# xxcclong/Distributed-CUDA-BFS

Measured on AMD Instinct MI355X. Metric: GTEPS (traversed edges/sec) on RMAT-26 + soc-LiveJournal1 at 1/2/4/8 MI355X, higher is better.
Workload: dtype uint8 levels (int32 on read)

## Files before the change

csrc/backend/cpu_backend.cpp:

```cpp
#include <algorithm>
#include <chrono>
#include <cstdlib>
#include <cstring>
#include <utility>
#include <vector>

#include "dbfs/backend.hpp"

namespace dbfs {
namespace {

inline void put_level(lvl_t* wide, uint8_t* narrow, int64_t i, lvl_t level, uint8_t base) {
  if (narrow) narrow[i] = static_cast<uint8_t>(base + (level <= kNarrowMaxLevel ? level : kNarrowMaxLevel + 1));
  else wide[i] = level;
}

inline bool test_bit(const word_t* bm, uint64_t v) { return (bm[v >> 6] >> (v & 63)) & 1ull; }
inline word_t gather_bytes(uint8_t* p) {
  word_t bits = 0;
  for (int b = 0; b < 64; ++b)
    if (p[b]) bits |= 1ull << b;
  if (bits) std::memset(p, 0, 64);
  return bits;
}
// ... 618 lines not shown
  void encode_hub_cols(const vid_t* col, int64_t nnz, const uint32_t* hub_idx, vid_t* out) override {
    for (int64_t e = 0; e < nnz; ++e) out[e] = hub_idx[col[e]] != 0xFFFFFFFFu ? (kHubFlag | hub_idx[col[e]]) : col[e];
  }
  void nz_word_counts(const eid_t* ro, int64_t rows, int64_t words, eid_t* counts) override {
    for (int64_t w = 0; w < words; ++w) {
      eid_t c = 0;
      for (int64_t v = w * 64; v < std::min<int64_t>(rows, (w + 1) * 64); ++v) c += ro[v + 1] > ro[v] ? 1 : 0;
      counts[w] = c;
    }
  }
  void nz_fill(const eid_t* ro, const vid_t* head, int64_t rows, const eid_t* pref, eid_t* nz_ro,
               vid_t* nz_head) override {
    int64_t k = 0;
    for (int64_t v = 0; v < rows; ++v) {
      if (ro[v + 1] > ro[v]) {
        nz_ro[k] = ro[v];
        nz_head[k] = head[v];
        ++k;
      }
    }
    nz_ro[k] = rows > 0 ? ro[rows] : 0;
    (void)pref;
  }
  void nz_records(const eid_t* ro, const vid_t* head, int64_t rows, const eid_t* pref, NzRec* rec,
                  eid_t* unit_base) override {
    const int64_t nunits = div_up(std::max<int64_t>(rows, 1), kUnitVertices);
    for (int64_t u = 0; u <= nunits; ++u) unit_base[u] = ro[std::min<int64_t>(u * kUnitVertices, rows)];
    int64_t k = 0;
    for (int64_t v = 0; v < rows; ++v) {
      if (ro[v + 1] > ro[v]) {
        rec[k].off = static_cast<uint32_t>(ro[v] - unit_base[v / kUnitVertices]);
        rec[k].head = head[v];
        ++k;
      }
    }
    (void)pref;
  }
  int64_t select_hubs(const uint32_t* deg, int64_t n, uint32_t min_deg, vid_t* hub_vertex,
                      uint32_t* hub_idx) override {
    int64_t k = 0;
    for (int64_t v = 0; v < n; ++v) {
      if (deg[v] >= min_deg) {
        hub_vertex[k] = static_cast<vid_t>(v);
        hub_idx[v] = static_cast<uint32_t>(k++);
      } else {
        hub_idx[v] = 0xFFFFFFFFu;
      }
    }
    return k;
  }
  void hub_gather(const HubGatherArgs& a) override {
    if (a.ctrl && (a.ctrl->done || a.ctrl->dir != 'B')) return;
    for (int64_t w = 0; w < div_up(a.g.nhubs, 64); ++w) {
      word_t m = 0;
      int64_t d = 0;
// ... 193 lines not shown
```

csrc/backend/hip_backend.cpp:

```cpp
#include <hip/hip_runtime.h>

#include <chrono>
#include <cstdlib>
#include <cstring>
#include <string>
#include <vector>

#include "dbfs/backend.hpp"
#include "../kernels/launch.hpp"

namespace dbfs {

#define HIP_CHECK(expr)                                                                              \
  do {                                                                                               \
    hipError_t e_ = (expr);                                                                          \
    if (e_ != hipSuccess)                                                                            \
      ::dbfs::raise_error(__FILE__, __LINE__, std::string("HIP error ") + hipGetErrorString(e_) +    \
                                                  " in " #expr);                                     \
  } while (0)

namespace {

class HipBackend final : public Backend {
 public:
// ... 241 lines not shown
  void validate_levels(const ValidateArgs& a) override { on(); kern::validate_levels(a, st_); chk(); }
  void compute_parents(const ParentArgs& a) override { on(); kern::compute_parents(a, st_); chk(); }
  void degrees_u32(const eid_t* ro, int64_t rows, uint32_t* out) override {
    on();
    kern::degrees_u32(ro, rows, out, st_);
    chk();
  }
  void row_heads(const eid_t* ro, const vid_t* col, int64_t rows, vid_t* head, const uint32_t* hub_idx) override {
    on();
    kern::row_heads(ro, col, rows, head, hub_idx, st_);
    chk();
  }

  void encode_hub_cols(const vid_t* col, int64_t nnz, const uint32_t* hub_idx, vid_t* out) override {
    on();
    kern::encode_hub_cols(col, nnz, hub_idx, out, st_);
    chk();
  }
  void nz_word_counts(const eid_t* ro, int64_t rows, int64_t words, eid_t* counts) override {
    on();
    kern::nz_word_counts(ro, rows, words, counts, st_);
    chk();
  }
  void nz_records(const eid_t* ro, const vid_t* head, int64_t rows, const eid_t* pref, NzRec* rec,
                  eid_t* unit_base) override {
    on();
    kern::nz_records(ro, head, rows, div_up(rows, kWordBits), pref, rec, unit_base, st_);
    chk();
  }
  void nz_fill(const eid_t* ro, const vid_t* head, int64_t rows, const eid_t* pref, eid_t* nz_ro,
               vid_t* nz_head) override {
    on();
    kern::nz_fill(ro, head, rows, div_up(rows, kWordBits), pref, nz_ro, nz_head, st_);
    chk();
  }
  int64_t select_hubs(const uint32_t* deg, int64_t n, uint32_t min_deg, vid_t* hub_vertex,
                      uint32_t* hub_idx) override {
    on();
    const int64_t words = div_up(std::max<int64_t>(n, 1), kWordBits);
    eid_t* cnt = nullptr;
    HIP_CHECK(hipMalloc(&cnt, static_cast<size_t>(words + 1) * sizeof(eid_t)));
    HIP_CHECK(hipMemsetAsync(cnt, 0, static_cast<size_t>(words + 1) * sizeof(eid_t), st_));
    kern::hub_count(deg, n, min_deg, cnt, st_);
    chk();
    exclusive_scan(cnt, words);
    kern::hub_assign(deg, n, min_deg, cnt, hub_vertex, hub_idx, st_);
    chk();
    eid_t h = 0;
    HIP_CHECK(hipMemcpyAsync(&h, cnt + words, sizeof(h), hipMemcpyDeviceToHost, st_));
    HIP_CHECK(hipStreamSynchronize(st_));
// ... 124 lines not shown
```

csrc/engine/engine.cpp:

```cpp
#include <algorithm>
#include <chrono>
#include <cstdio>
#include <cstdlib>
#include <cstring>
#include <thread>
#include <vector>

#include "dbfs/engine.hpp"
#include "dbfs/shard_reader.hpp"
#include "dbfs/trace.hpp"
#include "spin.hpp"

namespace dbfs {

Mode parse_mode(const std::string& s) {
  if (s == "ref" || s == "reference") return Mode::Ref;
  if (s == "td" || s == "topdown" || s == "top-down") return Mode::TopDown;
  if (s == "bu" || s == "bottomup" || s == "bottom-up") return Mode::BottomUp;
  if (s == "do" || s == "diropt" || s == "direction-optimizing" || s == "hybrid") return Mode::DirOpt;
  if (s == "simple" || s == "status") return Mode::Simple;
  if (s == "scan") return Mode::Scan;
  throw Error("unknown mode '" + s + "' (expected ref|td|bu|do|simple|scan)");
}

// ... 237 lines not shown
  auto g = from_edges(be, comm, part, rank, es.m, es.u.data(), es.v.data(), es.local_edges());
  g->ingest_ = {es.byte_begin, es.byte_end, es.local_edges()};
  return g;
}

ShardView DeviceGraph::view() const {
  ShardView v;
  v.row_off = row_off_.data();
  v.col = col_.data();
  v.n = part_.n;
  v.lo = lo_;
  v.rows = rows_;
  v.nnz = nnz_;
  v.head = head_.data();
  v.hub_vertex = hub_vertex_.data();
  v.nhubs = nhubs_;
  v.hub_col = hub_col_.data();
  v.hub_bits = hub_bits_.data();
  v.hub_deg = hub_deg_.data();
  v.nz_pref = nz_pref_.data();
  v.nz_row_off = nz_row_off_.data();
  v.nz_head = nz_head_.data();
  v.nz_rec = nz_rec_.data();
  v.unit_base = unit_base_.data();
  if (td_nhubs_ > 0) {
    v.td_col = td_col_.data();
    v.td_hub_vertex = td_hub_vertex_.data();
    v.td_nhubs = td_nhubs_;
  }
  return v;
}

HostCSR DeviceGraph::to_host() const {
  HostCSR h;
  h.n = part_.n;
  h.row_lo = lo_;
  h.rows = rows_;
  h.input_edges = input_edges_;
  h.row_off.resize(static_cast<size_t>(rows_ + 1));
  h.col.resize(static_cast<size_t>(nnz_));
  be_->to_host(h.row_off.data(), row_off_.data(), h.row_off.size() * sizeof(eid_t));
  if (nnz_) be_->to_host(h.col.data(), col_.data(), h.col.size() * sizeof(vid_t));
  return h;
}

std::vector<eid_t> DeviceGraph::degrees_of(const std::vector<int64_t>& local_rows) const {
  std::vector<eid_t> out;
  out.reserve(local_rows.size());
  for (int64_t r : local_rows) {
    DBFS_CHECK(r >= 0 && r < rows_, "row out of range");
    eid_t a[2];
    be_->to_host(a, row_off_.data() + r, sizeof(a));
    out.push_back(a[1] - a[0]);
  }
  return out;
}

static uint32_t hub_min_degree(const std::vector<uint32_t>& deg, int64_t cap) {
  constexpr uint32_t kCapDeg = 1u << 20;
  std::vector<int64_t> hist(kCapDeg + 1, 0);
  for (uint32_t d : deg) ++hist[std::min(d, kCapDeg)];
  int64_t acc = 0;
  uint32_t best = 0;
  for (uint32_t d = kCapDeg; d >= 1; --d) {
    acc += hist[d];
    if (acc > cap) break;
// ... 91 lines not shown
  hub_sorted_ = true;
}

void DeviceGraph::build_heads(const uint32_t* hub_idx) {
  if (head_.size() < static_cast<size_t>(std::max<int64_t>(rows_, 1)))
    head_ = DBuf<vid_t>(*be_, static_cast<size_t>(std::max<int64_t>(rows_, 1)));
  be_->row_heads(row_off_.data(), col_.data(), rows_, head_.data(), hub_idx);
  build_nz_view();
  be_->synchronize();
}

void DeviceGraph::build_nz_view() {
  const int64_t words = div_up(std::max<int64_t>(rows_, 1), kWordBits);
  nz_pref_ = DBuf<eid_t>(*be_, static_cast<size_t>(words + 1));
  be_->memset_async(nz_pref_.data(), 0, nz_pref_.bytes());
  be_->nz_word_counts(row_off_.data(), rows_, words, nz_pref_.data());
  be_->exclusive_scan(nz_pref_.data(), words);
  eid_t nzrows = 0;
  be_->to_host(&nzrows, nz_pref_.data() + words, sizeof(eid_t));
  nz_row_off_ = DBuf<eid_t>(*be_, static_cast<size_t>(nzrows + 1));
  nz_head_ = DBuf<vid_t>(*be_, static_cast<size_t>(std::max<eid_t>(nzrows, 1)));
  be_->nz_fill(row_off_.data(), head_.data(), rows_, nz_pref_.data(), nz_row_off_.data(), nz_head_.data());
  nz_rec_ = DBuf<NzRec>();
  unit_base_ = DBuf<eid_t>();
  if (rows_ <= 0) return;
  const int64_t nunits = div_up(rows_, kUnitVertices);
  unit_base_ = DBuf<eid_t>(*be_, static_cast<size_t>(nunits + 1));
  nz_rec_ = DBuf<NzRec>(*be_, static_cast<size_t>(std::max<eid_t>(nzrows, 1)));
  be_->nz_records(row_off_.data(), head_.data(), rows_, nz_pref_.data(), nz_rec_.data(), unit_base_.data());
  std::vector<eid_t> ub(static_cast<size_t>(nunits + 1));
  be_->to_host(ub.data(), unit_base_.data(), ub.size() * sizeof(eid_t));
  for (int64_t u = 0; u < nunits; ++u)
    if (ub[static_cast<size_t>(u + 1)] - ub[static_cast<size_t>(u)] >= (eid_t(1) << 32)) {
      nz_rec_ = DBuf<NzRec>();
      unit_base_ = DBuf<eid_t>();
      break;
    }
}


Engine::Engine(DeviceGraph& g, Comm& comm, const EngineOptions& opt)
    : g_(g), comm_(comm), be_(g.backend()), opt_(opt), part_(g.partition()), fault_(FaultSpec::from_env()) {
  DBFS_CHECK(comm.size() == part_.nranks, "communicator size does not match the partition");
  DBFS_CHECK(comm.rank() == g.rank(), "communicator rank does not match the shard");
  comm_.bind_backend(&be_);
  total_directed_ = comm_.sum_host(g.nnz());
  level_ = DBuf<lvl_t>(be_, static_cast<size_t>(std::max<int64_t>(g.rows(), 1)));
  be_.fill_level(level_.data(), g.rows(), kUnreached);
}

Engine::~Engine() {
  if (mailbox_host_) be_.free_mapped(mailbox_host_);
  for (auto& seg : rec_segs_) be_.free_mapped(seg.first);
  if (stats_mb_host_) be_.free_mapped(stats_mb_host_);
}


// ... 724 lines not shown
```

csrc/include/dbfs/backend.hpp:

```cpp
#pragma once

#include <atomic>
#include <cstddef>
#include <functional>
#include <memory>
#include <string>
#include <utility>

#include "dbfs/common.hpp"
#include "dbfs/rmat.hpp"

namespace dbfs {

enum class DeviceKind { CPU, HIP };


struct alignas(8) NzRec {
  uint32_t off;
  vid_t head;
};

struct ShardView {
  const eid_t* row_off = nullptr;
  const vid_t* col = nullptr;
  int64_t n = 0, lo = 0, rows = 0, nnz = 0;
  const vid_t* head = nullptr;
  const vid_t* hub_vertex = nullptr;
  int64_t nhubs = 0;
  const vid_t* hub_col = nullptr;
  const eid_t* nz_pref = nullptr;
  const eid_t* nz_row_off = nullptr;
  const vid_t* nz_head = nullptr;
  const struct NzRec* nz_rec = nullptr;
  const eid_t* unit_base = nullptr;
  const vid_t* td_col = nullptr;
  const vid_t* td_hub_vertex = nullptr;
  int64_t td_nhubs = 0;
  const word_t* hub_bits = nullptr;
  const uint32_t* hub_deg = nullptr;
};

#ifndef DBFS_TD_MAX_HUBS_LOG2
#define DBFS_TD_MAX_HUBS_LOG2 16
#endif
constexpr int64_t kTdMaxHubs = int64_t(1) << DBFS_TD_MAX_HUBS_LOG2;

#ifndef DBFS_MAX_HUBS
#define DBFS_MAX_HUBS ((int64_t(1) << 19) - (int64_t(1) << 12))
#endif
constexpr int64_t kMaxHubs = DBFS_MAX_HUBS;
constexpr vid_t kHubFlag = 0x80000000u;
constexpr int kSortedRowMax = 4096;
constexpr uint8_t kNarrowUnreached = 0xFF;
constexpr int kNarrowMaxLevel = 62;
constexpr int kNarrowEpochs = 4;

// ... 604 lines not shown
  virtual bool device_checks_enabled() const { return false; }
  virtual uint64_t take_device_check() { return 0; }
  virtual void inject_device_check() {}
  virtual void status_expand(const StatusArgs& a) = 0;
  virtual void bitmap_or(word_t* dst, const word_t* src, int64_t words) = 0;
  virtual void ref_expand(const RefExpandArgs& a) = 0;
  virtual void ref_accept(const RefAcceptArgs& a) = 0;
  virtual void scan_relax(const ScanBfsArgs& a) = 0;
  virtual void scan_count(const ScanBfsArgs& a) = 0;
  virtual void scan_bounds(const ScanBfsArgs& a) = 0;
  virtual void scan_assign(const ScanBfsArgs& a) = 0;
  virtual void validate_levels(const ValidateArgs& a) = 0;
  virtual void compute_parents(const ParentArgs& a) = 0;

  virtual void degrees_u32(const eid_t* row_off, int64_t rows, uint32_t* out) = 0;
  virtual void sort_neighbors(const eid_t* row_off, vid_t* col, int64_t rows, const uint32_t* key_deg) = 0;
  virtual void sort_rows_by_id(const eid_t* row_off, vid_t* col, int64_t rows, int64_t n) = 0;
  virtual void row_heads(const eid_t* row_off, const vid_t* col, int64_t rows, vid_t* head,
                         const uint32_t* hub_idx = nullptr) = 0;
  virtual void nz_word_counts(const eid_t* row_off, int64_t rows, int64_t words, eid_t* counts) = 0;
  virtual void nz_fill(const eid_t* row_off, const vid_t* head, int64_t rows, const eid_t* nz_pref, eid_t* nz_row_off,
                       vid_t* nz_head) = 0;
  virtual void nz_records(const eid_t* row_off, const vid_t* head, int64_t rows, const eid_t* nz_pref, NzRec* rec,
                          eid_t* unit_base) = 0;
  virtual void encode_hub_cols(const vid_t* col, int64_t nnz, const uint32_t* hub_idx, vid_t* out) = 0;
  virtual int64_t select_hubs(const uint32_t* deg_all, int64_t n, uint32_t min_deg, vid_t* hub_vertex,
                              uint32_t* hub_idx) = 0;

  virtual void gen_count_degrees(const GenParams& p, int64_t lo, int64_t rows, eid_t* deg) = 0;
  virtual void exclusive_scan(eid_t* data, int64_t n) = 0;
  virtual void gen_fill(const GenParams& p, int64_t lo, int64_t rows, eid_t* cursor, vid_t* col) = 0;
  virtual void route_edges_count(const vid_t* u, const vid_t* v, int64_t m, int64_t part, int nranks,
                                 int64_t* counts) = 0;
  virtual void route_edges_fill(const vid_t* u, const vid_t* v, int64_t m, int64_t part, int nranks,
                                int64_t* cursor, uint64_t* out) = 0;
  virtual void entries_count(const uint64_t* e, int64_t k, int64_t lo, eid_t* deg) = 0;
  virtual void entries_fill(const uint64_t* e, int64_t k, int64_t lo, eid_t* cursor, vid_t* col) = 0;
  virtual void reached_degree_sum(const ShardView& g, const lvl_t* level, int64_t* out2) = 0;
  virtual void degree_moments(const ShardView& g, int64_t* out2) = 0;
  virtual void widen_levels(const uint8_t* in, lvl_t* out, int64_t n, uint8_t base) = 0;

 protected:
  std::function<void(double)> wait_watch_;
  double wait_period_ = 0.05;
  std::atomic<int64_t> live_bytes_{0}, peak_bytes_{0};
};

// ... 45 lines not shown
```

csrc/include/dbfs/engine.hpp:

```cpp
#pragma once

#include <memory>
#include <string>
#include <utility>
#include <vector>

#include "dbfs/backend.hpp"
#include "dbfs/comm.hpp"
#include "dbfs/graph.hpp"
#include "dbfs/partition.hpp"

namespace dbfs {

enum class Mode { Ref, TopDown, BottomUp, DirOpt, Simple, Scan };
Mode parse_mode(const std::string& s);
const char* mode_name(Mode m);

class DeviceGraph {
 public:
  static std::unique_ptr<DeviceGraph> from_host(Backend& be, const HostCSR& csr, const Partition& part, int rank);
  static std::unique_ptr<DeviceGraph> generate(Backend& be, const GenParams& p, const Partition& part, int rank);
  static std::unique_ptr<DeviceGraph> from_edges(Backend& be, Comm& comm, const Partition& part, int rank,
                                                 int64_t input_edges, const vid_t* u, const vid_t* v,
                                                 int64_t m_local);
  static std::unique_ptr<DeviceGraph> from_file(Backend& be, Comm& comm, const std::string& path, int threads = 0);

  ShardView view() const;
  HostCSR to_host() const;
  Backend& backend() const { return *be_; }
  const Partition& partition() const { return part_; }
  int rank() const { return rank_; }
  int64_t n() const { return part_.n; }
  int64_t lo() const { return lo_; }
  int64_t rows() const { return rows_; }
  int64_t nnz() const { return nnz_; }
  int64_t input_edges() const { return input_edges_; }
  std::vector<eid_t> degrees_of(const std::vector<int64_t>& local_rows) const;
  void sort_neighbors_by_degree(Comm& comm, bool hubs = true, int64_t max_hubs = kMaxHubs, bool id_order = true,
                                bool td_hubs = true);
  bool hub_sorted() const { return hub_sorted_; }
  bool col_by_id() const { return col_by_id_; }
  double td_hub_share() const { return td_hub_share_; }
  bool rec_all() const { return rec_all_; }
  int64_t nhubs() const { return nhubs_; }
  struct IngestInfo {
    int64_t byte_begin = -1, byte_end = -1, edges = -1;
  };
  const IngestInfo& ingest() const { return ingest_; }

 private:
  IngestInfo ingest_;
  Backend* be_ = nullptr;
  Partition part_;
  int rank_ = 0;
  int64_t lo_ = 0, rows_ = 0, nnz_ = 0, input_edges_ = 0;
  bool hub_sorted_ = false;
  bool col_by_id_ = false;
  int64_t nhubs_ = 0;
  bool rec_all_ = false;
  void build_heads(const uint32_t* hub_idx = nullptr);
  DBuf<vid_t> head_, hub_vertex_, nz_head_, hub_col_, td_col_, td_hub_vertex_;
  double td_hub_share_ = 0.0;
  DBuf<uint32_t> hub_deg_;
  DBuf<word_t> hub_bits_;
  int64_t td_nhubs_ = 0;
  DBuf<eid_t> nz_pref_, nz_row_off_;
  DBuf<NzRec> nz_rec_;
  DBuf<eid_t> unit_base_;
  void build_nz_view();
  DBuf<eid_t> row_off_;
  DBuf<vid_t> col_;
};

struct EngineOptions {
  Mode mode = Mode::DirOpt;
  double alpha = 40.0;
  double beta = 384.0;
  int bu_lane_limit = 16;
  int bu_whole_units = 0;
  int bu_small_waves = 0;
  int64_t td_byte_edges = int64_t(1) << 22;
  static constexpr bool td_direct = true;
  int64_t td_direct_edges = int64_t(1) << 16;
  int64_t td_bin_edges = int64_t(1) << 21;
  int64_t td_bin_min_rows = int64_t(1) << 26;
  static constexpr int64_t td_bin_log2_bins = 8;
  int64_t td_unvis_edges = int64_t(1) << 22;
  double td_unvis_vis_frac = 0.6;
  double td_unvis_max_density = 0.5;
  int64_t td_split_edges = int64_t(1) << 23;
// ... 196 lines not shown
```

csrc/kernels/bu_kernels.hip:

```cpp
#include <hip/hip_runtime.h>

#include <algorithm>
#include <cstdio>
#include <cstdlib>
#include <type_traits>

#include "kernel_common.hpp"
#include "launch.hpp"
#include "level_device.hpp"
#include "wave.hpp"

namespace dbfs {
namespace kern {
namespace {

__device__ __forceinline__ void unit_stats_store(long long cnt, long long deg, int64_t unit, int64_t* unit_cnt,
                                                 int64_t* unit_deg) {
  __shared__ long long s_c[kUnitWaves], s_d[kUnitWaves];
  cnt = wave_sum(cnt);
  deg = wave_sum(deg);
  const int wv = threadIdx.x >> 6;
  if (lane_id() == 0) {
    s_c[wv] = cnt;
    s_d[wv] = deg;
  }
  __syncthreads();
  if (threadIdx.x == 0) {
    long long c = 0, d = 0;
#pragma unroll
    for (int k = 0; k < kUnitWaves; ++k) {
      c += s_c[k];
      d += s_d[k];
    }
    unit_cnt[unit] = c;
    unit_deg[unit] = d;
  }
}

constexpr int kBuBatch = 4;
constexpr int kCutLevels = 1, kCutClaims = 2;

constexpr int kBuQueue = 64;
static_assert(kBuQueue <= kWave, "one queued row per lane per flush");

#ifdef DBFS_BU_STATS
__device__ unsigned long long g_bu_stats[8];
#define BU_STAT(i, x)                                                   \
  do {                                                                  \
    const unsigned long long v_ = (x);                                  \
    if (lane_id() == 0 && v_) atomicAdd(&g_bu_stats[i], v_);            \
  } while (0)
#else
#define BU_STAT(i, x) \
  do {                \
  } while (0)
#endif

template <bool kHub>
__device__ __forceinline__ bool bu_probe(const word_t* __restrict__ fr, const word_t* s_hub, vid_t u) {
  if constexpr (kHub) {
    const vid_t hb = u & ~kHubFlag;
    return (u & kHubFlag) ? ((s_hub[hb >> 6] >> (hb & 63)) & 1ull) : test_bit(fr, u);
  } else {
    return test_bit(fr, u);
  }
// ... 190 lines not shown
      loc = j * 64 + bit;
      if (kRec || nz_ro) {
        const int64_t k = a.g.nz_pref[w0 + j] + __popcll(~a.zdeg[w0 + j] & ((1ull << bit) - 1ull));
        if constexpr (kRec) {
          const NzRec r = nz_rec[k];
          const uint32_t end = k + 1 < u_nzend ? nz_rec[k + 1].off : u_span;
          rs = u_base + r.off;
          len = end - r.off;
          u = r.head;
        } else {
          rs = nz_ro[k];
          len = static_cast<uint32_t>(nz_ro[k + 1] - rs);
          u = a.g.nz_head[k];
        }
      } else {
        const int64_t v = w0 * 64 + loc;
        rs = ro[v];
        len = static_cast<uint32_t>(ro[v + 1] - rs);
        if (head) u = head[v];
      }
    }
  };
  const int nb = (total + kWave - 1) / kWave;
  int n_loc;
  eid_t n_rs;
  uint32_t n_len;
  vid_t n_u;
  fetch(0, n_loc, n_rs, n_len, n_u);
  if (!head) n_u = n_len ? col[n_rs] : 0u;
  int cnt32 = 0;
  eid_t q_base = 0;
  bool q_span_ok = false;
  int qn = 0;
  if constexpr (kQueue > 0) {
    const int64_t wend = min(w0 + nw, (a.g.rows + kWordBits - 1) / kWordBits);
    if constexpr (kRec) {
      q_base = u_base;
      q_span_ok = true;
    } else if (nz_ro) {
      q_base = nz_ro[a.g.nz_pref[w0]];
      q_span_ok = nz_ro[a.g.nz_pref[wend]] - q_base < (eid_t(1) << 32);
    } else {
      const int64_t vend = min(wend * 64, a.g.rows);
      q_base = ro[w0 * 64];
      q_span_ok = ro[vend] - q_base < (eid_t(1) << 32);
    }
  }
  auto settle = [&](bool f, int l, eid_t r0, eid_t r1) {
    if (f) {
      store_level(a.level, a.level8, w0 * 64 + l, a.new_level, a.narrow_base);
      cnt32 += 1;
      deg += r1 - r0;
      __hip_atomic_fetch_or(s_res + (l >> 6), 1ull << (l & 63), __ATOMIC_RELAXED, __HIP_MEMORY_SCOPE_WAVEFRONT);
    }
  };
  auto flush = [&]() {
    __builtin_amdgcn_fence(__ATOMIC_RELEASE, "wavefront");
    __builtin_amdgcn_wave_barrier();
    int ql = 0;
    eid_t qrs = 0, qe = 0;
    if (lane < qn) {
      const unsigned long long ent = s_q[lane];
      ql = static_cast<int>(ent & 0xFFFu);
      qrs = q_base + static_cast<eid_t>(ent >> 32);
      qe = qrs + static_cast<eid_t>((ent >> 12) & 0xFFFFFu);
    }
    __builtin_amdgcn_fence(__ATOMIC_RELEASE, "wavefront");
    __builtin_amdgcn_wave_barrier();
    const bool f = bu_scan_row<kHub, (kCut != 0)>(a, qrs, qe, lane >= qn, s_hub, cut);
    settle(lane < qn && f, ql, qrs, qe);
    qn = 0;
  };
  for (int b = 0; b < nb; ++b) {
    const int loc = n_loc;
    const eid_t rs = n_rs, e = n_rs + n_len;
    const vid_t u0 = n_u;
    fetch(b + 1, n_loc, n_rs, n_len, n_u);
    bool found = false;
    bool cut_row = false;
    if constexpr (kCut) {
      cut_row = cut && !(u0 & kHubFlag) && e - rs <= static_cast<eid_t>(kSortedRowMax);
      if (rs < e && !cut_row) found = bu_probe<kHub>(fr, s_hub, u0);
    } else {
      if (rs < e) found = bu_probe<kHub>(fr, s_hub, u0);
    }
    BU_STAT(0, 1);
    BU_STAT(1, __popcll(__ballot(loc >= 0)));
    BU_STAT(2, __popcll(__ballot(found)));
    if (!head) n_u = n_len ? col[n_rs] : 0u;
    if constexpr (kQueue > 0) {
      const bool need = !found && e - rs > 1 && !cut_row;
      const bool fits = q_span_ok && e - rs < (eid_t(1) << 20);
      const bool direct = __popcll(__ballot(need && fits)) > kQueue;
      const bool inplace = need && (direct || !fits);
      if (__ballot(inplace)) {
        const bool f = bu_scan_row<kHub, (kCut != 0)>(a, rs, e, found || !inplace, s_hub, cut);
        if (inplace) found = f;
      }
      settle(found, loc, rs, e);
      const bool defer = need && !inplace;
      const unsigned long long dm = __ballot(defer);
      const int k = __popcll(dm);
      if (qn + k > kQueue) flush();
      if (defer)
        s_q[qn + mask_rank(dm)] = (static_cast<unsigned long long>(rs - q_base) << 32) |
                                  (static_cast<unsigned long long>(e - rs) << 12) | static_cast<unsigned>(loc);
      qn += k;
    } else {
      found = bu_scan_row<kHub, (kCut != 0)>(a, rs, e, found || cut_row, s_hub, cut) && !cut_row;
      BU_STAT(7, __popcll(__ballot(found)));
      settle(found, loc, rs, e);
    }
  }
  if constexpr (kQueue > 0) {
    if (qn) flush();
  }
  cnt += cnt32;
  __builtin_amdgcn_fence(__ATOMIC_RELEASE, "wavefront");
  __builtin_amdgcn_wave_barrier();
  if (lane < nw) {
    const word_t res = s_res[lane] | pw;
    a.new_frontier[w0 + lane] = res;
    if (res) a.visited[w0 + lane] = ~um | res;
  }
  take_pre();
}

__global__ __launch_bounds__(kUnitThreads) void bu_kernel(BuArgs a) {
  __shared__ word_t s_res[kUnitWaves * kWaveWords];
  if (a.ctrl && (a.ctrl->done || a.ctrl->dir != 'B')) return;
  stamp_level_start(a.ctrl);
  long long cnt = 0, deg = 0;
  const int wave = __builtin_amdgcn_readfirstlane(static_cast<int>(threadIdx.x >> 6));
  const int64_t w0 = static_cast<int64_t>(blockIdx.x) * kUnitWords + wave * kWaveWords;
// ... 476 lines not shown
```

csrc/kernels/graph_sort.hip:

```cpp
#include <hip/hip_runtime.h>

#include <algorithm>

#include "launch.hpp"
#include "wave.hpp"

namespace dbfs {
namespace kern {
namespace {

using namespace dev;

constexpr int kBlock = 256;
constexpr int kMaxLds = kSortedRowMax;

__device__ __forceinline__ unsigned long long sort_key(uint32_t deg, vid_t v) {
  return (static_cast<unsigned long long>(0xFFFFFFFFu - deg) << 32) | v;
}
__device__ __forceinline__ unsigned long long row_key(const uint32_t* __restrict__ key_deg, vid_t v) {
  return sort_key(key_deg ? key_deg[v] : 0u, v);
}

__global__ __launch_bounds__(kBlock) void degrees_kernel(const eid_t* __restrict__ ro, int64_t rows,
                                                        uint32_t* __restrict__ out) {
// ... 170 lines not shown
  const bool nz = v < rows && ro[v + 1] > ro[v];
  const unsigned long long m = __ballot(nz);
  if (lane_id() == 0) counts[w] = __popcll(m);
}

__global__ __launch_bounds__(kBlock) void nz_fill_kernel(const eid_t* __restrict__ ro, const vid_t* __restrict__ head,
                                                        int64_t rows, int64_t words, const eid_t* __restrict__ pref,
                                                        eid_t* __restrict__ nz_ro, vid_t* __restrict__ nz_head) {
  const int64_t w = static_cast<int64_t>(blockIdx.x) * (kBlock / kWave) + (threadIdx.x >> 6);
  if (w >= words) return;
  const int64_t v = w * kWave + lane_id();
  const bool nz = v < rows && ro[v + 1] > ro[v];
  const unsigned long long m = __ballot(nz);
  if (nz) {
    const int64_t k = pref[w] + mask_rank(m);
    nz_ro[k] = ro[v];
    nz_head[k] = head[v];
  }
  if (w == words - 1 && lane_id() == 0) nz_ro[pref[words]] = ro[rows];
}

__global__ __launch_bounds__(kBlock) void nz_rec_kernel(const eid_t* __restrict__ ro, const vid_t* __restrict__ head,
                                                       int64_t rows, int64_t words, const eid_t* __restrict__ pref,
                                                       NzRec* __restrict__ rec) {
  const int64_t w = static_cast<int64_t>(blockIdx.x) * (kBlock / kWave) + (threadIdx.x >> 6);
  if (w >= words) return;
  const int64_t v = w * kWave + lane_id();
  const bool nz = v < rows && ro[v + 1] > ro[v];
  const unsigned long long m = __ballot(nz);
  if (nz) {
    const int64_t k = pref[w] + mask_rank(m);
    NzRec r;
    r.off = static_cast<uint32_t>(ro[v] - ro[(v / kUnitVertices) * kUnitVertices]);
    r.head = head[v];
    rec[k] = r;
  }
}

__global__ __launch_bounds__(kBlock) void unit_base_kernel(const eid_t* __restrict__ ro, int64_t rows, int64_t nunits,
                                                          eid_t* __restrict__ unit_base) {
  const int64_t u = static_cast<int64_t>(blockIdx.x) * kBlock + threadIdx.x;
  if (u <= nunits) unit_base[u] = ro[min(u * kUnitVertices, rows)];
}

__global__ __launch_bounds__(kBlock) void hub_count_kernel(const uint32_t* __restrict__ deg, int64_t n,
                                                          uint32_t min_deg, eid_t* __restrict__ cnt) {
  const int64_t v = static_cast<int64_t>(blockIdx.x) * kBlock + threadIdx.x;
  const unsigned long long m = __ballot(v < n && deg[v] >= min_deg);
  if (lane_id() == 0 && (v >> 6) * 64 < n) cnt[v >> 6] = __popcll(m);
}

__global__ __launch_bounds__(kBlock) void hub_assign_kernel(const uint32_t* __restrict__ deg, int64_t n,
                                                           uint32_t min_deg, const eid_t* __restrict__ cnt,
                                                           vid_t* __restrict__ hub_vertex,
                                                           uint32_t* __restrict__ hub_idx) {
  const int64_t v = static_cast<int64_t>(blockIdx.x) * kBlock + threadIdx.x;
  const bool hub = v < n && deg[v] >= min_deg;
  const unsigned long long m = __ballot(hub);
// ... 12 lines not shown
  row_heads_kernel<<<static_cast<unsigned>((rows + kBlock - 1) / kBlock), kBlock, 0, st>>>(row_off, col, rows, head,
                                                                                          hub_idx);
}

void encode_hub_cols(const vid_t* col, int64_t nnz, const uint32_t* hub_idx, vid_t* out, hipStream_t st) {
  if (nnz <= 0) return;
  encode_hub_cols_kernel<<<static_cast<unsigned>(std::min<int64_t>((nnz + kBlock - 1) / kBlock, 1 << 16)), kBlock, 0,
                           st>>>(col, nnz, hub_idx, out);
}

void nz_word_counts(const eid_t* row_off, int64_t rows, int64_t words, eid_t* counts, hipStream_t st) {
  if (words <= 0) return;
  nz_count_kernel<<<static_cast<unsigned>((words + 3) / 4), kBlock, 0, st>>>(row_off, rows, words, counts);
}

void nz_fill(const eid_t* row_off, const vid_t* head, int64_t rows, int64_t words, const eid_t* nz_pref,
             eid_t* nz_row_off, vid_t* nz_head, hipStream_t st) {
  if (words <= 0) return;
  nz_fill_kernel<<<static_cast<unsigned>((words + 3) / 4), kBlock, 0, st>>>(row_off, head, rows, words, nz_pref,
                                                                          nz_row_off, nz_head);
}

void nz_records(const eid_t* row_off, const vid_t* head, int64_t rows, int64_t words, const eid_t* nz_pref,
                NzRec* rec, eid_t* unit_base, hipStream_t st) {
  if (rows <= 0) return;
  const int64_t nunits = (rows + kUnitVertices - 1) / kUnitVertices;
  unit_base_kernel<<<static_cast<unsigned>((nunits + 1 + kBlock - 1) / kBlock), kBlock, 0, st>>>(row_off, rows, nunits,
                                                                                                unit_base);
  nz_rec_kernel<<<static_cast<unsigned>((words + 3) / 4), kBlock, 0, st>>>(row_off, head, rows, words, nz_pref, rec);
}

void hub_count(const uint32_t* deg, int64_t n, uint32_t min_deg, eid_t* cnt, hipStream_t st) {
  if (n <= 0) return;
  hub_count_kernel<<<static_cast<unsigned>((n + kBlock - 1) / kBlock), kBlock, 0, st>>>(deg, n, min_deg, cnt);
}

void hub_assign(const uint32_t* deg, int64_t n, uint32_t min_deg, const eid_t* cnt, vid_t* hub_vertex,
                uint32_t* hub_idx, hipStream_t st) {
  if (n <= 0) return;
  hub_assign_kernel<<<static_cast<unsigned>((n + kBlock - 1) / kBlock), kBlock, 0, st>>>(deg, n, min_deg, cnt,
                                                                                        hub_vertex, hub_idx);
}

void degrees_u32(const eid_t* row_off, int64_t rows, uint32_t* out, hipStream_t st) {
  if (rows <= 0) return;
  degrees_kernel<<<static_cast<unsigned>((rows + kBlock - 1) / kBlock), kBlock, 0, st>>>(row_off, rows, out);
}

void sort_neighbors(const eid_t* row_off, vid_t* col, int64_t rows, const uint32_t* key_deg, int64_t* list,
                    unsigned long long* count, hipStream_t st) {
  if (rows <= 0) return;
  sort_short_rows_kernel<<<8192, kBlock, 0, st>>>(row_off, col, rows, key_deg);
// ... 22 lines not shown
```

csrc/kernels/launch.hpp:

```cpp
#pragma once

#include <hip/hip_runtime.h>

#include "dbfs/backend.hpp"

namespace dbfs {
namespace kern {

void fill_level(lvl_t* level, int64_t n, lvl_t value, hipStream_t st);
bool zero_fill(void* p, size_t bytes, hipStream_t st);
void set_bit(word_t* bm, int64_t bit, hipStream_t st);
void level_ctrl_init(LevelCtrl* c, const LevelCtrl& init, hipStream_t st);
void publish_stats(const int64_t* stats, StatsMailbox* mb, int64_t seq, hipStream_t st);
void init_run(const InitRunArgs& a, hipStream_t st);
void update_frontier(const UpdateArgs& a, hipStream_t st);
void scan_units(const ScanArgs& a, hipStream_t st);
void zero_degree_mask(const ZeroDegArgs& a, hipStream_t st);
void compact_frontier(const CompactArgs& a, hipStream_t st);
void td_expand(const TdArgs& a, hipStream_t st);
void td_sparse(const TdSparseArgs& a, hipStream_t st);
void td_sparse_apply(const TdSparseArgs& a, hipStream_t st);
void direct_prewait(const DirectExchange& x, hipStream_t st);
void direct_selftest(const DirectExchange& lists, const DirectExchange& end, int round, unsigned* err,
                     unsigned* ticket, hipStream_t st);
// ... 71 lines not shown
void scan_bounds(const ScanBfsArgs& a, hipStream_t st);
void scan_assign(const ScanBfsArgs& a, hipStream_t st);

void gen_count_degrees(const GenParams& p, int64_t lo, int64_t rows, eid_t* deg, hipStream_t st);
void gen_fill(const GenParams& p, int64_t lo, int64_t rows, eid_t* cursor, vid_t* col, hipStream_t st);
void route_edges_count(const vid_t* u, const vid_t* v, int64_t m, int64_t part, int nranks, int64_t* counts,
                       hipStream_t st);
void route_edges_fill(const vid_t* u, const vid_t* v, int64_t m, int64_t part, int nranks, int64_t* cursor,
                      uint64_t* out, hipStream_t st);
void entries_count(const uint64_t* e, int64_t k, int64_t lo, eid_t* deg, hipStream_t st);
void entries_fill(const uint64_t* e, int64_t k, int64_t lo, eid_t* cursor, vid_t* col, hipStream_t st);
int route_max_ranks();
int64_t scan_tmp_elems(int64_t n);
void exclusive_scan(eid_t* data, int64_t n, eid_t* tmp, hipStream_t st);
void validate_levels(const ValidateArgs& a, hipStream_t st);
void compute_parents(const ParentArgs& a, hipStream_t st);

void degrees_u32(const eid_t* row_off, int64_t rows, uint32_t* out, hipStream_t st);
void row_heads(const eid_t* row_off, const vid_t* col, int64_t rows, vid_t* head, const uint32_t* hub_idx,
               hipStream_t st);
void encode_hub_cols(const vid_t* col, int64_t nnz, const uint32_t* hub_idx, vid_t* out, hipStream_t st);
void nz_word_counts(const eid_t* row_off, int64_t rows, int64_t words, eid_t* counts, hipStream_t st);
void nz_records(const eid_t* row_off, const vid_t* head, int64_t rows, int64_t words, const eid_t* nz_pref,
                NzRec* rec, eid_t* unit_base, hipStream_t st);
void nz_fill(const eid_t* row_off, const vid_t* head, int64_t rows, int64_t words, const eid_t* nz_pref,
             eid_t* nz_row_off, vid_t* nz_head, hipStream_t st);
void hub_count(const uint32_t* deg, int64_t n, uint32_t min_deg, eid_t* cnt, hipStream_t st);
void hub_assign(const uint32_t* deg, int64_t n, uint32_t min_deg, const eid_t* cnt, vid_t* hub_vertex,
                uint32_t* hub_idx, hipStream_t st);
void sort_neighbors(const eid_t* row_off, vid_t* col, int64_t rows, const uint32_t* key_deg, int64_t* list,
                    unsigned long long* count, hipStream_t st);
void sort_rows_by_id(const eid_t* row_off, vid_t* col, int64_t rows, int64_t n, int64_t* list,
                     unsigned long long* count, vid_t* tmp, hipStream_t st);
void reached_degree_sum(const ShardView& g, const lvl_t* level, int64_t* out2, hipStream_t st);
void degree_moments(const ShardView& g, int64_t* out2, hipStream_t st);

}
}
```

csrc/python/module.cpp:

```cpp
#include <pybind11/numpy.h>
#include <pybind11/pybind11.h>
#include <pybind11/stl.h>

#include <chrono>
#include <cstring>

#include "dbfs/engine.hpp"
#include "dbfs/shard_reader.hpp"

namespace py = pybind11;
using namespace dbfs;

namespace {

template <class T>
py::array_t<T> to_numpy(const std::vector<T>& v) {
  py::array_t<T> a(static_cast<py::ssize_t>(v.size()));
  if (!v.empty()) std::memcpy(a.mutable_data(), v.data(), v.size() * sizeof(T));
  return a;
}

template <class T>
std::vector<T> from_numpy(const py::array_t<T, py::array::c_style | py::array::forcecast>& a) {
  std::vector<T> v(static_cast<size_t>(a.size()));
// ... 538 lines not shown
            return std::shared_ptr<DeviceGraph>(DeviceGraph::from_file(*be, comm, path, threads));
          },
          py::arg("backend"), py::arg("comm"), py::arg("path"), py::arg("threads") = 0, py::keep_alive<0, 1>())
      .def_property_readonly("n", &DeviceGraph::n)
      .def_property_readonly("lo", &DeviceGraph::lo)
      .def_property_readonly("rows", &DeviceGraph::rows)
      .def_property_readonly("nnz", &DeviceGraph::nnz)
      .def_property_readonly("input_edges", &DeviceGraph::input_edges)
      .def_property_readonly("rank", &DeviceGraph::rank)
      .def_property_readonly("partition", &DeviceGraph::partition)
      .def("to_host", &DeviceGraph::to_host, py::call_guard<py::gil_scoped_release>())
      .def("sort_neighbors_by_degree", &DeviceGraph::sort_neighbors_by_degree, py::arg("comm"),
           py::arg("hubs") = true, py::arg("max_hubs") = kMaxHubs, py::arg("id_order") = true,
           py::arg("td_hubs") = true,
           py::call_guard<py::gil_scoped_release>())
      .def_property_readonly("col_by_id", &DeviceGraph::col_by_id)
      .def_property_readonly("td_hub_share", &DeviceGraph::td_hub_share)
      .def_property_readonly("hub_sorted", &DeviceGraph::hub_sorted)
      .def_property_readonly("nhubs", &DeviceGraph::nhubs)
      .def_property_readonly("ingest",
                             [](const DeviceGraph& g) {
                               return py::make_tuple(g.ingest().byte_begin, g.ingest().byte_end, g.ingest().edges);
                             })
      .def("degrees_of", &DeviceGraph::degrees_of);

  py::class_<RunResult>(m, "RunResult")
      .def_readonly("source", &RunResult::source)
      .def_readonly("ms", &RunResult::ms)
      .def_readonly("reached", &RunResult::reached)
      .def_readonly("edges", &RunResult::edges)
      .def_readonly("depth", &RunResult::depth)
      .def_readonly("gteps", &RunResult::gteps)
      .def_readonly("mispredicts", &RunResult::mispredicts)
      .def_property_readonly("chains",
                             [](const RunResult& r) {
                               py::list out;
                               for (const auto& c : r.chains)
                                 out.append(py::make_tuple(c.level, std::string(1, c.form), c.cap, c.gather, c.push, c.unvis, c.split, c.cut));
                               return out;
                             })
      .def("level_dicts", &level_dicts);

  py::class_<Engine, std::shared_ptr<Engine>>(m, "Engine")
      .def(py::init([](std::shared_ptr<DeviceGraph> g, std::shared_ptr<Comm> c, const std::string& mode, double alpha,
                       double beta, int bu_lane_limit, bool phase_timing, bool force_exchange) {
             EngineOptions o;
             o.mode = parse_mode(mode);
// ... 111 lines not shown
```

Baseline: 1586.

## Walk nonzero-row records directly in bottom-up unit scan when unvisited density is high

Adds a per-nonzero-row uint16 local index array built alongside the NzRec records. The bottom-up unit kernel gets a second path: when the count of unvisited rows in a unit is at least half the unit's nonzero rows, it streams the records contiguously with prefetch and masks each row by the unvisited bitmap, instead of compacting unvisited rows first and fetching them indirectly. This removes per-row indirect fetches and compaction on dense units. In exchange it costs extra device memory for the loc array, and sparse-frontier lanes go idle on masked rows. The density threshold is a compile-time ratio.

```diff
diff --git a/csrc/backend/cpu_backend.cpp b/csrc/backend/cpu_backend.cpp
--- a/csrc/backend/cpu_backend.cpp
+++ b/csrc/backend/cpu_backend.cpp
@@ -664,7 +664,7 @@
     nz_ro[k] = rows > 0 ? ro[rows] : 0;
     (void)pref;
   }
-  void nz_records(const eid_t* ro, const vid_t* head, int64_t rows, const eid_t* pref, NzRec* rec,
+  void nz_records(const eid_t* ro, const vid_t* head, int64_t rows, const eid_t* pref, NzRec* rec, uint16_t* loc,
                   eid_t* unit_base) override {
     const int64_t nunits = div_up(std::max<int64_t>(rows, 1), kUnitVertices);
     for (int64_t u = 0; u <= nunits; ++u) unit_base[u] = ro[std::min<int64_t>(u * kUnitVertices, rows)];
@@ -673,6 +673,7 @@
       if (ro[v + 1] > ro[v]) {
         rec[k].off = static_cast<uint32_t>(ro[v] - unit_base[v / kUnitVertices]);
         rec[k].head = head[v];
+        loc[k] = static_cast<uint16_t>(v % kUnitVertices);
         ++k;
       }
     }
diff --git a/csrc/backend/hip_backend.cpp b/csrc/backend/hip_backend.cpp
--- a/csrc/backend/hip_backend.cpp
+++ b/csrc/backend/hip_backend.cpp
@@ -287,10 +287,10 @@
     kern::nz_word_counts(ro, rows, words, counts, st_);
     chk();
   }
-  void nz_records(const eid_t* ro, const vid_t* head, int64_t rows, const eid_t* pref, NzRec* rec,
+  void nz_records(const eid_t* ro, const vid_t* head, int64_t rows, const eid_t* pref, NzRec* rec, uint16_t* loc,
                   eid_t* unit_base) override {
     on();
-    kern::nz_records(ro, head, rows, div_up(rows, kWordBits), pref, rec, unit_base, st_);
+    kern::nz_records(ro, head, rows, div_up(rows, kWordBits), pref, rec, loc, unit_base, st_);
     chk();
   }
   void nz_fill(const eid_t* ro, const vid_t* head, int64_t rows, const eid_t* pref, eid_t* nz_ro,
diff --git a/csrc/engine/engine.cpp b/csrc/engine/engine.cpp
--- a/csrc/engine/engine.cpp
+++ b/csrc/engine/engine.cpp
@@ -283,6 +283,7 @@
   v.nz_row_off = nz_row_off_.data();
   v.nz_head = nz_head_.data();
   v.nz_rec = nz_rec_.data();
+  v.nz_loc = nz_loc_.data();
   v.unit_base = unit_base_.data();
   if (td_nhubs_ > 0) {
     v.td_col = td_col_.data();
@@ -303,6 +304,17 @@
   be_->to_host(h.row_off.data(), row_off_.data(), h.row_off.size() * sizeof(eid_t));
   if (nnz_) be_->to_host(h.col.data(), col_.data(), h.col.size() * sizeof(vid_t));
   return h;
+}
+
+std::vector<uint16_t> DeviceGraph::debug_nz_loc() const {
+  std::vector<uint16_t> out;
+  if (!nz_loc_.data() || !nz_rec_.data()) return out;
+  const int64_t words = div_up(std::max<int64_t>(rows_, 1), kWordBits);
+  eid_t nzrows = 0;
+  be_->to_host(&nzrows, nz_pref_.data() + words, sizeof(eid_t));
+  out.resize(static_cast<size_t>(nzrows));
+  if (nzrows) be_->to_host(out.data(), nz_loc_.data(), out.size() * sizeof(uint16_t));
+  return out;
 }
 
 std::vector<eid_t> DeviceGraph::degrees_of(const std::vector<int64_t>& local_rows) const {
@@ -440,17 +452,21 @@
   nz_head_ = DBuf<vid_t>(*be_, static_cast<size_t>(std::max<eid_t>(nzrows, 1)));
   be_->nz_fill(row_off_.data(), head_.data(), rows_, nz_pref_.data(), nz_row_off_.data(), nz_head_.data());
   nz_rec_ = DBuf<NzRec>();
+  nz_loc_ = DBuf<uint16_t>();
   unit_base_ = DBuf<eid_t>();
   if (rows_ <= 0) return;
   const int64_t nunits = div_up(rows_, kUnitVertices);
   unit_base_ = DBuf<eid_t>(*be_, static_cast<size_t>(nunits + 1));
   nz_rec_ = DBuf<NzRec>(*be_, static_cast<size_t>(std::max<eid_t>(nzrows, 1)));
-  be_->nz_records(row_off_.data(), head_.data(), rows_, nz_pref_.data(), nz_rec_.data(), unit_base_.data());
+  nz_loc_ = DBuf<uint16_t>(*be_, static_cast<size_t>(std::max<eid_t>(nzrows, 1)));
+  be_->nz_records(row_off_.data(), head_.data(), rows_, nz_pref_.data(), nz_rec_.data(), nz_loc_.data(),
+                  unit_base_.data());
   std::vector<eid_t> ub(static_cast<size_t>(nunits + 1));
   be_->to_host(ub.data(), unit_base_.data(), ub.size() * sizeof(eid_t));
   for (int64_t u = 0; u < nunits; ++u)
     if (ub[static_cast<size_t>(u + 1)] - ub[static_cast<size_t>(u)] >= (eid_t(1) << 32)) {
       nz_rec_ = DBuf<NzRec>();
+      nz_loc_ = DBuf<uint16_t>();
       unit_base_ = DBuf<eid_t>();
       break;
     }
diff --git a/csrc/include/dbfs/backend.hpp b/csrc/include/dbfs/backend.hpp
--- a/csrc/include/dbfs/backend.hpp
+++ b/csrc/include/dbfs/backend.hpp
@@ -32,6 +32,7 @@
   const eid_t* nz_row_off = nullptr;
   const vid_t* nz_head = nullptr;
   const struct NzRec* nz_rec = nullptr;
+  const uint16_t* nz_loc = nullptr;
   const eid_t* unit_base = nullptr;
   const vid_t* td_col = nullptr;
   const vid_t* td_hub_vertex = nullptr;
@@ -682,7 +683,7 @@
   virtual void nz_fill(const eid_t* row_off, const vid_t* head, int64_t rows, const eid_t* nz_pref, eid_t* nz_row_off,
                        vid_t* nz_head) = 0;
   virtual void nz_records(const eid_t* row_off, const vid_t* head, int64_t rows, const eid_t* nz_pref, NzRec* rec,
-                          eid_t* unit_base) = 0;
+                          uint16_t* loc, eid_t* unit_base) = 0;
   virtual void encode_hub_cols(const vid_t* col, int64_t nnz, const uint32_t* hub_idx, vid_t* out) = 0;
   virtual int64_t select_hubs(const uint32_t* deg_all, int64_t n, uint32_t min_deg, vid_t* hub_vertex,
                               uint32_t* hub_idx) = 0;
diff --git a/csrc/include/dbfs/engine.hpp b/csrc/include/dbfs/engine.hpp
--- a/csrc/include/dbfs/engine.hpp
+++ b/csrc/include/dbfs/engine.hpp
@@ -36,6 +36,7 @@
   int64_t nnz() const { return nnz_; }
   int64_t input_edges() const { return input_edges_; }
   std::vector<eid_t> degrees_of(const std::vector<int64_t>& local_rows) const;
+  std::vector<uint16_t> debug_nz_loc() const;
   void sort_neighbors_by_degree(Comm& comm, bool hubs = true, int64_t max_hubs = kMaxHubs, bool id_order = true,
                                 bool td_hubs = true);
   bool hub_sorted() const { return hub_sorted_; }
@@ -66,6 +67,7 @@
   int64_t td_nhubs_ = 0;
   DBuf<eid_t> nz_pref_, nz_row_off_;
   DBuf<NzRec> nz_rec_;
+  DBuf<uint16_t> nz_loc_;
   DBuf<eid_t> unit_base_;
   void build_nz_view();
   DBuf<eid_t> row_off_;
diff --git a/csrc/kernels/bu_kernels.hip b/csrc/kernels/bu_kernels.hip
--- a/csrc/kernels/bu_kernels.hip
+++ b/csrc/kernels/bu_kernels.hip
@@ -41,6 +41,13 @@
 constexpr int kCutLevels = 1, kCutClaims = 2;
 
 constexpr int kBuQueue = 64;
+#ifndef DBFS_REC_WALK_NUM
+#define DBFS_REC_WALK_NUM 1
+#endif
+#ifndef DBFS_REC_WALK_DEN
+#define DBFS_REC_WALK_DEN 2
+#endif
+constexpr int kRecWalkNum = DBFS_REC_WALK_NUM, kRecWalkDen = DBFS_REC_WALK_DEN;
 static_assert(kBuQueue <= kWave, "one queued row per lane per flush");
 
 #ifdef DBFS_BU_STATS
@@ -277,12 +284,24 @@
     }
   };
   const int nb = (total + kWave - 1) / kWave;
-  int n_loc;
-  eid_t n_rs;
-  uint32_t n_len;
-  vid_t n_u;
-  fetch(0, n_loc, n_rs, n_len, n_u);
-  if (!head) n_u = n_len ? col[n_rs] : 0u;
+  constexpr bool kRecWalk = kRec && kWords == kUnitWords;
+  bool rec_walk = false;
+  int64_t k0 = 0;
+  int nrec = 0;
+  if constexpr (kRecWalk) {
+    const int64_t row_words = (a.g.rows + kWordBits - 1) / kWordBits;
+    k0 = static_cast<int64_t>(readlane64(static_cast<unsigned long long>(a.g.nz_pref[min(w0, row_words)]), 0));
+    nrec = static_cast<int>(min(max(u_nzend - k0, int64_t(0)), static_cast<int64_t>(kUnitVertices)));
+    rec_walk = a.g.nz_loc != nullptr && total * kRecWalkDen >= nrec * kRecWalkNum;
+  }
+  int n_loc = -1;
+  eid_t n_rs = 0;
+  uint32_t n_len = 0;
+  vid_t n_u = 0;
+  if (!rec_walk) {
+    fetch(0, n_loc, n_rs, n_len, n_u);
+    if (!head) n_u = n_len ? col[n_rs] : 0u;
+  }
   int cnt32 = 0;
   eid_t q_base = 0;
   bool q_span_ok = false;
@@ -326,11 +345,7 @@
     settle(lane < qn && f, ql, qrs, qe);
     qn = 0;
   };
-  for (int b = 0; b < nb; ++b) {
-    const int loc = n_loc;
-    const eid_t rs = n_rs, e = n_rs + n_len;
-    const vid_t u0 = n_u;
-    fetch(b + 1, n_loc, n_rs, n_len, n_u);
+  auto step = [&](int loc, eid_t rs, eid_t e, vid_t u0, auto&& ahead) {
     bool found = false;
     bool cut_row = false;
     if constexpr (kCut) {
@@ -342,7 +357,7 @@
     BU_STAT(0, 1);
     BU_STAT(1, __popcll(__ballot(loc >= 0)));
     BU_STAT(2, __popcll(__ballot(found)));
-    if (!head) n_u = n_len ? col[n_rs] : 0u;
+    ahead();
     if constexpr (kQueue > 0) {
       const bool need = !found && e - rs > 1 && !cut_row;
       const bool fits = q_span_ok && e - rs < (eid_t(1) << 20);
@@ -365,6 +380,57 @@
       found = bu_scan_row<kHub, (kCut != 0)>(a, rs, e, found || cut_row, s_hub, cut) && !cut_row;
       BU_STAT(7, __popcll(__ballot(found)));
       settle(found, loc, rs, e);
+    }
+  };
+  if (rec_walk) {
+    if constexpr (kRecWalk) {
+      const NzRec* __restrict__ rp = nz_rec + k0;
+      const uint16_t* __restrict__ lp = a.g.nz_loc + k0;
+      const int nrb = (nrec + kWave - 1) / kWave;
+      uint32_t c_off, n_off;
+      vid_t c_u, n_hd;
+      int c_l, n_l;
+      auto load = [&](int b, uint32_t& off, vid_t& hd, int& l) {
+        off = u_span;
+        hd = 0;
+        l = 0;
+        const uint32_t i = static_cast<uint32_t>(b * kWave + lane);
+        if (i < static_cast<uint32_t>(nrec)) {
+          const NzRec r = rp[i];
+          off = r.off;
+          hd = r.head;
+          l = lp[i];
+        }
+      };
+      load(0, c_off, c_u, c_l);
+      load(1, n_off, n_hd, n_l);
+      for (int b = 0; b < nrb; ++b) {
+        const bool act = b * kWave + lane < nrec;
+        DBFS_DCHECK(!act || k0 + b * kWave + lane < u_nzend, 12, k0 + b * kWave + lane);
+        DBFS_DCHECK(!act || c_l < kUnitVertices, 13, c_l);
+        const uint32_t nx = static_cast<uint32_t>(__builtin_amdgcn_readfirstlane(static_cast<int>(n_off)));
+        const uint32_t dn = static_cast<uint32_t>(__shfl_down(static_cast<int>(c_off), 1, kWave));
+        const uint32_t end = lane == kWave - 1 ? nx : dn;
+        const word_t uw = static_cast<word_t>(__shfl(static_cast<long long>(um), (c_l >> 6) & (kWave - 1), kWave));
+        const bool live = act && ((uw >> (c_l & 63)) & 1ull);
+        const int loc = live ? c_l : -1;
+        const eid_t rs = live ? u_base + c_off : 0, e = live ? u_base + end : 0;
+        const vid_t u0 = c_u;
+        c_off = n_off;
+        c_u = n_hd;
+        c_l = n_l;
+        step(loc, rs, e, u0, [&]() { load(b + 2, n_off, n_hd, n_l); });
+      }
+    }
+  } else {
+    for (int b = 0; b < nb; ++b) {
+      const int loc = n_loc;
+      const eid_t rs = n_rs, e = n_rs + n_len;
+      const vid_t u0 = n_u;
+      fetch(b + 1, n_loc, n_rs, n_len, n_u);
+      step(loc, rs, e, u0, [&]() {
+        if (!head) n_u = n_len ? col[n_rs] : 0u;
+      });
     }
   }
   if constexpr (kQueue > 0) {
diff --git a/csrc/kernels/graph_sort.hip b/csrc/kernels/graph_sort.hip
--- a/csrc/kernels/graph_sort.hip
+++ b/csrc/kernels/graph_sort.hip
@@ -216,7 +216,7 @@
 
 __global__ __launch_bounds__(kBlock) void nz_rec_kernel(const eid_t* __restrict__ ro, const vid_t* __restrict__ head,
                                                        int64_t rows, int64_t words, const eid_t* __restrict__ pref,
-                                                       NzRec* __restrict__ rec) {
+                                                       NzRec* __restrict__ rec, uint16_t* __restrict__ loc) {
   const int64_t w = static_cast<int64_t>(blockIdx.x) * (kBlock / kWave) + (threadIdx.x >> 6);
   if (w >= words) return;
   const int64_t v = w * kWave + lane_id();
@@ -228,6 +228,7 @@
     r.off = static_cast<uint32_t>(ro[v] - ro[(v / kUnitVertices) * kUnitVertices]);
     r.head = head[v];
     rec[k] = r;
+    loc[k] = static_cast<uint16_t>(v % kUnitVertices);
   }
 }
 
@@ -286,12 +287,13 @@
 }
 
 void nz_records(const eid_t* row_off, const vid_t* head, int64_t rows, int64_t words, const eid_t* nz_pref,
-                NzRec* rec, eid_t* unit_base, hipStream_t st) {
+                NzRec* rec, uint16_t* loc, eid_t* unit_base, hipStream_t st) {
   if (rows <= 0) return;
   const int64_t nunits = (rows + kUnitVertices - 1) / kUnitVertices;
   unit_base_kernel<<<static_cast<unsigned>((nunits + 1 + kBlock - 1) / kBlock), kBlock, 0, st>>>(row_off, rows, nunits,
                                                                                                 unit_base);
-  nz_rec_kernel<<<static_cast<unsigned>((words + 3) / 4), kBlock, 0, st>>>(row_off, head, rows, words, nz_pref, rec);
+  nz_rec_kernel<<<static_cast<unsigned>((words + 3) / 4), kBlock, 0, st>>>(row_off, head, rows, words, nz_pref, rec,
+                                                                           loc);
 }
 
 void hub_count(const uint32_t* deg, int64_t n, uint32_t min_deg, eid_t* cnt, hipStream_t st) {
diff --git a/csrc/kernels/launch.hpp b/csrc/kernels/launch.hpp
--- a/csrc/kernels/launch.hpp
+++ b/csrc/kernels/launch.hpp
@@ -117,7 +117,7 @@
 void encode_hub_cols(const vid_t* col, int64_t nnz, const uint32_t* hub_idx, vid_t* out, hipStream_t st);
 void nz_word_counts(const eid_t* row_off, int64_t rows, int64_t words, eid_t* counts, hipStream_t st);
 void nz_records(const eid_t* row_off, const vid_t* head, int64_t rows, int64_t words, const eid_t* nz_pref,
-                NzRec* rec, eid_t* unit_base, hipStream_t st);
+                NzRec* rec, uint16_t* loc, eid_t* unit_base, hipStream_t st);
 void nz_fill(const eid_t* row_off, const vid_t* head, int64_t rows, int64_t words, const eid_t* nz_pref,
              eid_t* nz_row_off, vid_t* nz_head, hipStream_t st);
 void hub_count(const uint32_t* deg, int64_t n, uint32_t min_deg, eid_t* cnt, hipStream_t st);
diff --git a/csrc/python/module.cpp b/csrc/python/module.cpp
--- a/csrc/python/module.cpp
+++ b/csrc/python/module.cpp
@@ -584,7 +584,13 @@
                              [](const DeviceGraph& g) {
                                return py::make_tuple(g.ingest().byte_begin, g.ingest().byte_end, g.ingest().edges);
                              })
-      .def("degrees_of", &DeviceGraph::degrees_of);
+      .def("degrees_of", &DeviceGraph::degrees_of)
+      .def("debug_nz_loc", [](const DeviceGraph& g) {
+        const std::vector<uint16_t> v = g.debug_nz_loc();
+        py::array_t<uint16_t> out(static_cast<py::ssize_t>(v.size()));
+        if (!v.empty()) std::memcpy(out.mutable_data(), v.data(), v.size() * sizeof(uint16_t));
+        return out;
+      });
 
   py::class_<RunResult>(m, "RunResult")
       .def_readonly("source", &RunResult::source)
```

Measured after the change: 1699 (median of 6 runs). 7.1% higher.
